# tyler-a-cox/fftvis

Hardware: AMD Instinct MI355X
Metric: simulated visibilities/sec (baselines x freqs x times) at eps=6e-8 (higher is better)
Workload: dtype f64; 1 GPU; C3: hera350, 100000 sources, 128 freqs, 20 times, 61075 baselines, polarized table beam, type3 NUFFT eps=6e-08 upsampfac=2

## Files before the change

### fftvis_amd/csrc/fv_nufft.h

```cpp
#pragma once

#include "fv_eskernel.h"

#include <hip/hip_ext.h>

#include <algorithm>
#include <cstdlib>
#include <array>
#include <map>
#include <memory>

namespace fv {

inline bool debug_switch_old_fft() {
    static const bool v = std::getenv("FFTVIS_HIP_OLD_FFT") != nullptr;
    return v;
}
inline bool debug_switch_natural_order() {
    static const bool v = std::getenv("FFTVIS_HIP_NATURAL_ORDER") != nullptr;
    return v;
}

constexpr int BINLOG = 3;
constexpr int GROUP = 16;
// ... 1987 lines not shown
    int64_t items_per_xcd;
    int n2[3], no[3];
    int P[3], cnt[3];
    double h[3];
    double btc[3], xc[3];
    int64_t out_fg_stride;
    int64_t out_k_stride;
    int64_t out_pol_off[16];
    int accumulate;
    int herm;
    int basis, kk, ll, nbasis, ncoef_freq, f_first;
    int transpose_flipped, basis_part, negate_all;
    const int *ctab;
    int ctab_stride, ncc;
    int *err;
    int wt_k;
    double wt_zc, wt_zh;
    const void *wt_bz;
    int zd_n;
    double zd_h, zd_btc, zd_xc;
    void *gs;
    int gs_nf, gs_f0;
    int64_t gs_nbls;
    const double *tg_w;
};

__device__ inline double bessel_j_series(int k, double x) {
    double lead = 1.0;
    for (int i = 1; i <= k; ++i) lead *= 0.5 * x / (double)i;
    const double q = -0.25 * x * x;
// ... 7 lines not shown
}

__device__ inline cplx<double> wterm_factor(int k, double zc, double zh, double zq) {
    double sn, cs;
    sincos(zc * zq, &sn, &cs);
    const double mag = (k ? 2.0 : 1.0) * bessel_j_series(k, zh * zq);
    const cplx<double> e = {cs * mag, sn * mag};
    switch (k & 3) {
        case 0: return e;
        case 1: return {-e.im, e.re};
        case 2: return {-e.re, -e.im};
        default: return {e.im, -e.re};
    }
}

template <typename T, int DIM, bool HERM, int NR, bool ZD = false, bool WT = false, bool GRAD = false, bool TANGENT = false>
__global__ __launch_bounds__(INTERP_THREADS) void k_interp(
    const cplx<T> *__restrict__ grid, int64_t N, const T *__restrict__ bt0,
    const T *__restrict__ bt1, const T *__restrict__ bt2, const int *__restrict__ bl_idx,
    const signed char *__restrict__ flip, const double *__restrict__ scale, InterpArgs a,
    KerParams ker, cplx<T> *__restrict__ out, const cplx<T> *__restrict__ coef,
    const int *__restrict__ ant1, const int *__restrict__ ant2, const int *__restrict__ ustart,
    const int *__restrict__ upairs) {
    const int tid = threadIdx.x;
    const int g = tid & (GROUP - 1);
    const int lane_base = (tid & 63) & ~(GROUP - 1);
    constexpr int IPW = INTERP_THREADS / GROUP;
    const int64_t per_xcd = a.items_per_xcd;
    const int64_t item = (int64_t)(blockIdx.x & 7) * per_xcd + (int64_t)(blockIdx.x >> 3) * IPW + tid / GROUP;
    if ((int64_t)(blockIdx.x >> 3) * IPW + tid / GROUP >= per_xcd || item >= N * a.nfg) return;
    const int fg = (int)(item / N);
// ... 48 lines not shown
    double pr = 1.0 / den, pi_ = 0.0;
    if (ph != 0.0) {
        double sn, cs;
        sincos(ph, &sn, &cs);
        pi_ = pr * sn;
        pr = pr * cs;
    }

    const int64_t row_sz = (int64_t)a.P[0] * a.cnt[0];
    const int64_t slab_sz = DIM == 2 && a.ctab ? row_sz * a.ncc : row_sz * a.P[1] * a.cnt[1];
    const int64_t plane_sz = DIM == 3 ? slab_sz * a.P[2] * a.cnt[2] : slab_sz;
    const int nouter = DIM == 3 ? w : 1;
    constexpr int NSIDE = HERM ? 2 : 1;
    constexpr int NVAL = HERM ? 2 : 16;
    double vre[NSIDE][HERM ? NVAL : 1], vim[NSIDE][HERM ? NVAL : 1];
    int j0s[NSIDE][DIM], roffs[NSIDE][NR], gcols[NSIDE];
    T kvs[NSIDE][DIM];
#pragma unroll
    for (int side = 0; side < NSIDE; ++side) {
        const double sgn = side ? -1.0 : 1.0;
        int (&j0)[DIM] = j0s[side];
        T (&kv)[DIM] = kvs[side];
#pragma unroll
        for (int d = 0; d < DIM; ++d) {
            const double e = sgn * th[d] * a.n2[d] * (0.5 / M_PI) + 0.5 * a.no[d];
            int j = (int)ceil(e - 0.5 * w);
            j = max(0, min(a.no[d] - w, j));
            j0[d] = j;
            kv[d] = g < w ? es_eval<T>((T)((double)(j + g) - e), beta, c4) : T(0);
        }
        int (&roff)[NR] = roffs[side];
        {
            const int P1 = a.P[1], c1 = a.cnt[1];
            int q1 = j0[1] / P1, r1 = j0[1] - q1 * P1;
#pragma unroll
            for (int rr = 0; rr < NR; ++rr) {
                int posr = r1 * c1 + q1;
                if (DIM == 2 && a.ctab) {
                    const int t = a.ctab[(int64_t)fg * a.ctab_stride + posr];
                    if (t == 0 && rr < w && g == 0 && a.err) atomicAdd(a.err, 1);
                    posr = max(t - 1, 0);
                }
                roff[rr] = posr * (int)row_sz;
                const int inc = rr + 1 < w ? 1 : 0;
                r1 += inc;
                const int wrap = r1 == P1 ? 1 : 0;
                r1 = wrap ? 0 : r1;
                q1 += wrap;
            }
        }
        gcols[side] = out_pos(min(j0[0] + g, a.no[0] - 1), a.P[0], a.cnt[0]);
    }
#pragma unroll
    for (int side = 0; side < NSIDE; ++side) {
        const double sgn = side ? -1.0 : 1.0;
        const int (&j0)[DIM] = j0s[side];
        const T (&kv)[DIM] = kvs[side];
        const int (&roff)[NR] = roffs[side];
        const int gcol = gcols[side];
        T k1[NR];
#pragma unroll
        for (int r = 0; r < NR; ++r) k1[r] = __shfl(kv[1], lane_base + r, 64);
        const double pis = side ? -pi_ : pi_;
        constexpr int RUNROLL = HERM ? NVAL : 1;
#pragma unroll RUNROLL
        for (int r = 0; r < (HERM ? NVAL : a.tpol); ++r) {
            const cplx<T> *plane = grid + ((int64_t)fg * a.tpol + r) * (zd ? plane_sz * a.zd_n : plane_sz) + gcol;
            T sr = T(0), si = T(0);
            if (zd) {
                double er, ei, dr, di;
                sincos(sgn * thz, &di, &dr);
                sincos(-sgn * thz * (double)(a.zd_n / 2), &ei, &er);
                double ar_ = 0.0, ai_ = 0.0;
                for (int zk = 0; zk < a.zd_n; ++zk) {
                    const cplx<T> *slab = plane + (int64_t)zk * plane_sz;
                    cplx<T> v[NR];
#pragma unroll
                    for (int rr = 0; rr < NR; ++rr) v[rr] = slab[roff[rr]];
                    T tr = T(0), ti = T(0);
#pragma unroll
                    for (int rr = 0; rr < NR; ++rr) {
                        tr += v[rr].re * k1[rr];
                        ti += v[rr].im * k1[rr];
                    }
                    ar_ += (double)tr * er - (double)ti * ei;
                    ai_ += (double)tr * ei + (double)ti * er;
                    const double e2 = er * dr - ei * di;
                    ei = er * di + ei * dr;
                    er = e2;
                }
                sr = (T)ar_;
                si = (T)ai_;
            }
            for (int ro = 0; ro < (zd ? 0 : nouter); ++ro) {
                T k2 = T(1);
                const cplx<T> *slab = plane;
                if (DIM == 3) {
                    k2 = __shfl(kv[DIM - 1], lane_base + ro, 64);
                    slab += (int64_t)out_pos(j0[DIM - 1] + ro, a.P[DIM - 1], a.cnt[DIM - 1]) * slab_sz;
                }
                cplx<T> v[NR];
#pragma unroll
                for (int rr = 0; rr < NR; ++rr) v[rr] = slab[roff[rr]];
                T tr = T(0), ti = T(0);
#pragma unroll
                for (int rr = 0; rr < NR; ++rr) {
                    tr += v[rr].re * k1[rr];
                    ti += v[rr].im * k1[rr];
                }
                sr += tr * k2;
                si += ti * k2;
            }
            sr *= kv[0];
            si *= kv[0];
#pragma unroll
            for (int off = GROUP / 2; off > 0; off >>= 1) {
                sr += __shfl_xor(sr, off, 64);
                si += __shfl_xor(si, off, 64);
            }
            const double vr0 = (double)sr * pr - (double)si * pis;
            const double vi0 = (double)sr * pis + (double)si * pr;
// ... 179 lines not shown
        }
      }
    }
}

struct RowMaskArgs {
    int w, nfg, sides;
    int n2x, nox, Px, cntx, n2y, noy, Py, Qy;
    double hx, btcx, hy, btcy;
    int blk_log, nblk, nw, ctab_stride;
};
template <typename T>
__global__ void k_plan_rowmask(int64_t NU, const T *__restrict__ btx, const T *__restrict__ bty,
                               const int *__restrict__ bl_idx, const signed char *__restrict__ flip,
                               const int *__restrict__ ustart, const double *__restrict__ scale, RowMaskArgs a,
                               const int *__restrict__ ctab, unsigned long long *__restrict__ mask) {
    const int64_t item = (int64_t)blockIdx.x * blockDim.x + threadIdx.x;
    if (item >= NU * a.nfg * a.sides) return;
    const int side = (int)(item % a.sides);
    const int64_t rest = item / a.sides;
    const int fg = (int)(rest / NU);
    const int64_t ui = rest % NU;
    const int64_t kl = ustart ? ustart[ui] : ui;
    const int64_t k = bl_idx ? bl_idx[kl] : kl;
    const double sg = (flip && flip[kl]) ? -1.0 : 1.0, sgn = side ? -1.0 : 1.0, sc = scale[fg];
    int lo[2], hi[2];
    const double hh[2] = {a.hx, a.hy}, bc[2] = {a.btcx, a.btcy};
    const int n2[2] = {a.n2x, a.n2y}, no[2] = {a.nox, a.noy};
    const double b[2] = {(double)btx[k], (double)bty[k]};
#pragma unroll
    for (int d = 0; d < 2; ++d) {
        const double sv = sc * sg * b[d];
        const double th = hh[d] * (sv - sc * bc[d]);
        const double e = sgn * th * n2[d] * (0.5 / M_PI) + 0.5 * no[d];
        const double t = e - 0.5 * a.w, jc = ceil(t);
        const bool amb = jc - t < 1e-6 || jc - t > 1.0 - 1e-6;
        lo[d] = max(0, min(no[d] - a.w, (int)jc));
        hi[d] = lo[d] + a.w - 1;
        if (amb) {
            lo[d] = max(0, lo[d] - 1);
            hi[d] = min(no[d] - 1, hi[d] + 1);
        }
    }
    const int half = a.noy / 2;
    for (int cx = lo[0]; cx <= hi[0]; ++cx) {
        const int t = ctab[(int64_t)fg * a.ctab_stride + out_pos(cx, a.Px, a.cntx)];
        if (!t) continue;
        const int64_t blk = (t - 1) >> a.blk_log;
        for (int cy = lo[1]; cy <= hi[1]; ++cy) {
            const int l = cy - half;
            int pp = l % a.Py;
            if (pp < 0) pp += a.Py;
            const int ks = (l - pp) / a.Py;
            const int c = (ks < 0 ? ks + a.Qy : ks) >> 4;
            atomicOr(&mask[(((int64_t)fg * a.nblk + blk) * a.Py + pp) * a.nw + (c >> 6)], 1ull << (c & 63));
        }
    }
}

struct BasisTerm {
    const void *coef;
    const int *ant1, *ant2;
    int kk, ll, nbasis, nfreq, f_first;
    int part = 0, negate = 0;
    void *gs = nullptr;
    int gs_nf = 0, gs_f0 = 0;
    int64_t gs_nbls = 0;
};

struct WTerm {
    int k;
    double zc, zh;
// ... 51 lines not shown
    }
    int *col_err = nullptr;
    const unsigned long long *col_omask = nullptr;
    int col_omask_nblk = 0;
    double col_out_cells = 0;
    void arm_columns(const int *tab, const int *xtab, int tpol, int ncc, int *err = nullptr, const unsigned long long *omask = nullptr,
                     int omask_nblk = 0) {
        col_tab = tab && xtab && (dim == 2 || zdirect) && b_block_log() ? tab : nullptr;
        col_xtab = col_tab ? xtab : nullptr;
        col_tab_tpol = tpol;
        col_ncc = ncc;
        col_err = err;
        col_omask = col_tab ? omask : nullptr;
        col_omask_nblk = omask_nblk;
        col_out_cells = 0;
    }
    int ypass_cols_log() const {
        int tpr, rpw;
        rowfft_shape(geo.d[1], true, tpr, rpw);
        return ilog2_c(rpw);
    }
    void build_rowmask(int64_t NU, const T *btx, const T *bty, const int *bl_idx, const signed char *flip, const int *ustart,
                       const double *scale_dev, int nfg, bool both, const int *ctab, int ncc, unsigned long long *mask,
                       int nblk, int nw) const {
        const DimGeom &x = geo.d[0], &y = geo.d[1];
        RowMaskArgs a{};
        a.w = ker.w;
        a.nfg = nfg;
        a.sides = both ? 2 : 1;
        a.n2x = x.n2; a.nox = x.no; a.Px = x.sP(); a.cntx = x.cnt(); a.hx = x.h; a.btcx = x.btc;
        a.n2y = y.n2; a.noy = y.no; a.Py = y.P; a.Qy = y.Q; a.hy = y.h; a.btcy = y.btc;
        a.blk_log = ypass_cols_log();
        a.nblk = nblk;
        a.nw = nw;
        a.ctab_stride = x.nos();
        (void)ncc;
        const int64_t items = NU * nfg * a.sides;
        if (items == 0) return;
        hipLaunchKernelGGL(k_plan_rowmask<T>, dim3((unsigned)cdiv(items, 256)), dim3(256), 0, stream, NU, btx, bty, bl_idx,
                           flip, ustart, scale_dev, a, ctab, mask);
    }
    int xcols() const { return col_tab ? col_ncc : geo.d[0].nos(); }
    int b_block_log_public() const { return b_block_log(); }
    bool columns_possible() const { return (dim == 2 || zdirect) && b_block_log() != 0 && y_reads_columns() && !fused_possible(); }
    bool fused_possible() const;
    bool prepare_fused_gather(int64_t N, const T *btx, const T *bty, const int *bl_idx, const signed char *flip,
                              const double *scale_dev, int nfg, int tpol, cplx<T> *out, int64_t out_fg_stride,
                              int64_t out_k_stride, const int64_t *out_pol_off, int64_t targets_serial = 0,
                              cplx<T> *out_mate = nullptr);
    int64_t M = 0;
    int64_t geom_serial = 0;

    DevBuf i0u, fu, tile_of, binmeta, bin_start, i0s, fs, perm, slot_id, kw, scan_tot, scan_off, scan_tot2, scan_off2;
    const int *Mp = nullptr;
    int *oob_ptr = nullptr;
// ... 329 lines not shown
    int launch_spread(int ntrans, int tbegin, hipEvent_t e0, hipEvent_t e1, Nufft3 *mate);
    void buffer_cells(int64_t &c0, int64_t &c1) const;
    void fft(int ntrans, Nufft3 *mate = nullptr);
    bool gang_compatible(const Nufft3 &o) const {
        bool ok = dim == 2 && o.dim == 2 && M == o.M && ker.w == o.ker.w;
        for (int d = 0; d < 2 && ok; ++d)
            ok = geo.d[d].na == o.geo.d[d].na && geo.d[d].n2 == o.geo.d[d].n2 && geo.d[d].no == o.geo.d[d].no &&
                 geo.d[d].h == o.geo.d[d].h && geo.d[d].xc == o.geo.d[d].xc && geo.d[d].btc == o.geo.d[d].btc;
        return ok;
    }
    double fft_traffic_cells() const;
    double fft_flops() const {
        const DimGeom &x = geo.d[0], &y = geo.d[1], &z = geo.d[2];
        const double zin = dim > 2 ? z.na : 1;
        auto f = [](const DimGeom &g) { return 5.0 * g.n2 * std::log2((double)g.n2); };
        double c = zin * y.na * f(x) + zin * (double)xcols() * f(y);
        if (dim > 2 && !zdirect) c += (double)x.nos() * y.nos() * f(z);
        return c;
    }
    int64_t spread_cells() const {
        return dim == 2 ? order_cells : row_ext_ptr ? order_cells * geo.d[2].na : geo.cells_a();
    }
    void interp(int64_t N, const T *btx, const T *bty, const T *btz, const int *bl_idx,
                const signed char *flip, const double *scale_dev, int nfg, int tpol,
                cplx<T> *out, int64_t out_fg_stride, int64_t out_k_stride,
                const int64_t *out_pol_off, bool accumulate, const struct BasisTerm *basis = nullptr,
                int herm = 0, const int *ustart = nullptr, int64_t nuniq = 0, const int *upairs = nullptr,
                const struct WTerm *wt = nullptr, const struct TanTerm *tan = nullptr);

   private:
    void rowfft(const cplx<T> *in, cplx<T> *out, const DimGeom &g, const cplx<T> *twd,
// ... 275 lines not shown
        FV_HIP(hipFuncSetAttribute(reinterpret_cast<const void *>(&k_rowfft_dif<T>),
                                   hipFuncAttributeMaxDynamicSharedMemorySize, 160 * 1024));
    hipLaunchKernelGGL(k_rowfft_dif<T>, jobs, dim3(a.tpr * a.rpw), smem, stream, in, out, twd, a);
}

template <typename T>
double Nufft3<T>::fft_traffic_cells() const {
    const DimGeom &x = geo.d[0], &y = geo.d[1], &z = geo.d[2];
    const double zin = dim > 2 ? z.na : 1;
    int tpr, rpw;
    rowfft_shape(y, true, tpr, rpw);
    const double xo = col_tab ? (double)col_ncc : (double)x.no;
    const double ain = row_ext_ptr ? (double)order_cells : (double)x.na * y.na;
    double c = zin * (ain + xo * y.na);
    if (!y_reads_columns()) c += zin * 2.0 * x.no * y.na;
    c += zin * (xo * y.na + (last_fft_fused ? 0.0 : col_tab && col_omask && col_out_cells > 0 ? col_out_cells : xo * y.no));
    if (dim > 2 && !zdirect) c += (double)x.no * y.no * (z.na + z.no);
    return c;
}

template <typename T>
void Nufft3<T>::fft(int ntrans, Nufft3 *mate) {
    const DimGeom &x = geo.d[0], &y = geo.d[1], &z = geo.d[2];
    int64_t c0, c1;
    buffer_cells(c0, c1);
    buf1.reserve(sizeof(cplx<T>) * c1 * ntrans);
    cplx<T> *cur = buf0.as<cplx<T>>(), *oth = buf1.as<cplx<T>>();
    cplx<T> *cur1 = nullptr, *oth1 = nullptr;
    if (mate) {
        FV_REQUIRE(gang_compatible(*mate), "gang launch needs two plans of one geometry");
        mate->buf1.reserve(sizeof(cplx<T>) * c1 * ntrans);
        cur1 = mate->buf0.template as<cplx<T>>();
        oth1 = mate->buf1.template as<cplx<T>>();
    }
    const int64_t zin = dim > 2 ? z.na : 1;
    const int64_t np = (int64_t)ntrans * zin;
    const int64_t xp = b_pitch();
    const int blk = b_block_log();
    FV_REQUIRE(!col_tab || (blk && y_reads_columns() && !fused_active), "column plan: blocked B, column-mode y-pass, stand-alone gather");
    first_pass_ext = row_ext_ptr;
    rowfft(cur, oth, x, tw_cur[0], np, y.na, (int64_t)y.na * x.na, x.na, 1, xp, 0, nullptr, cur1, oth1, 0, blk);
    first_pass_ext = nullptr;
    std::swap(cur, oth);
    std::swap(cur1, oth1);
    if (y_reads_columns()) {
        rowfft(cur, oth, y, tw_cur[1], np, xp, (int64_t)y.na * xp, 1, xp, 0, xcols(),
               fused_active ? &fused_args : nullptr, cur1, oth1, blk, 0);
        std::swap(cur, oth);
        std::swap(cur1, oth1);
    } else {
        dim3 tg((unsigned)cdiv(x.nos(), 32), (unsigned)cdiv(y.na, 32), (unsigned)np);
        hipLaunchKernelGGL(k_transpose<T>, tg, dim3(256), 0, stream, cur, oth, y.na, x.nos());
        if (mate) hipLaunchKernelGGL(k_transpose<T>, tg, dim3(256), 0, stream, cur1, oth1, y.na, x.nos());
        rowfft(oth, cur, y, tw_cur[1], np, x.nos(), (int64_t)x.nos() * y.na, y.na, 1, 0, 0, nullptr,
               oth1, cur1);
    }
    if (dim > 2 && !zdirect) {
        const int64_t nc = (int64_t)x.nos() * y.nos();
        rowfft(cur, oth, z, tw_cur[2], ntrans, nc, (int64_t)z.na * nc, 1, nc);
        std::swap(cur, oth);
// ... 153 lines not shown
        bt[i] = bts[map[i]];
    }
    FV_REQUIRE((int64_t)a.P[0] * a.cnt[0] * (col_tab ? (int64_t)col_ncc : (int64_t)a.P[1] * a.cnt[1]) < ((int64_t)1 << 31),
               "transform output slab of 2^31 elements or more: beyond the gather's 32-bit row offsets");
    a.out_fg_stride = out_fg_stride;
    a.out_k_stride = out_k_stride;
    for (int r = 0; r < 16; ++r) a.out_pol_off[r] = out_pol_off ? out_pol_off[r] : 0;
    a.accumulate = accumulate ? 1 : 0;
    if (col_tab) {
        FV_REQUIRE(gdim == 2, "column plan: 2-D transforms (or 3-D ones with the direct third dimension)");
        a.ctab = col_tab;
        a.ctab_stride = geo.d[0].nos();
        a.ncc = col_ncc;
        a.err = col_err;
    }
    a.herm = herm;
    a.transpose_flipped = transpose_flipped ? 1 : 0;
    a.wt_k = -1;
    if (wt) {
        FV_REQUIRE(dim == 2 && wt->bz && wt->k >= 0, "height terms ride on 2-D transforms");
        a.wt_k = wt->k;
        a.wt_zc = wt->zc;
        a.wt_zh = wt->zh;
        a.wt_bz = wt->bz;
    }
    const int64_t items = N * nfg;
    constexpr int IPW = INTERP_THREADS / GROUP;
    a.items_per_xcd = cdiv(cdiv(items, 8), IPW) * IPW;
    const dim3 grid((unsigned)(8 * (a.items_per_xcd / IPW)));
    const bool r9 = ker.w <= 9;
// ... 23 lines not shown
    }
    if (tan) {
        FV_REQUIRE(!basis && !a.gs, "tangent epilogue: no basis term and no gradient epilogue");
        a.tg_w = tan->w;
        kern = gdim == 2 ? (herm ? (r9 ? k_interp<T, 2, true, 9, false, false, false, true> : k_interp<T, 2, true, 16, false, false, false, true>)
                                 : (r9 ? k_interp<T, 2, false, 9, false, false, false, true> : k_interp<T, 2, false, 16, false, false, false, true>))
                         : (herm ? (r9 ? k_interp<T, 3, true, 9, false, false, false, true> : k_interp<T, 3, true, 16, false, false, false, true>)
                                 : (r9 ? k_interp<T, 3, false, 9, false, false, false, true> : k_interp<T, 3, false, 16, false, false, false, true>));
        if (zd)
            kern = herm ? (r9 ? k_interp<T, 2, true, 9, true, false, false, true> : k_interp<T, 2, true, 16, true, false, false, true>)
                        : (r9 ? k_interp<T, 2, false, 9, true, false, false, true> : k_interp<T, 2, false, 16, true, false, false, true>);
        if (wt)
            kern = herm ? (r9 ? k_interp<T, 2, true, 9, false, true, false, true> : k_interp<T, 2, true, 16, false, true, false, true>)
                        : (r9 ? k_interp<T, 2, false, 9, false, true, false, true> : k_interp<T, 2, false, 16, false, true, false, true>);
    }
    hipLaunchKernelGGL(kern, grid, dim3(INTERP_THREADS), 0, stream, (const cplx<T> *)grid_out, N, bt[0], bt[1], bt[2],
                       bl_idx, flip, scale_dev, a, ker, out, coef, ant1, ant2, ustart, upairs);
}

}
```

### fftvis_amd/csrc/fv_sim.h

```cpp
#pragma once

#include <atomic>
#include <chrono>
#include <cstdio>
#include <thread>
#include "fv_nufft.h"
#include <unordered_map>

#include <algorithm>
#include <array>
#include <cstdlib>
#include <memory>

namespace fv {

constexpr double SPEED_OF_LIGHT = 299792458.0;

struct BeamDesc {
    int kind;
    int order;
    double diameter;
    double js[8];
    double ps;
    const void *table;
// ... 1739 lines not shown
    int64_t out_f_stride = 0;
    int out_shared = 0;
    int adjoint_path = 0;
    int last_adjoint_path = 0;
    virtual void sync() = 0;
    virtual void stats(double *v, int n) = 0;
    virtual void reset_stats() = 0;
    virtual void enable_timing(int on) = 0;
    virtual void timing(double *ms, int n) = 0;
};

enum { TM_SPREAD = 0, TM_FFT, TM_INTERP, TM_STRENGTHS, TM_PREP, TM_COUNT };
enum {
    ST_SPREAD_LAUNCHES = 0, ST_SPREAD_CELLS, ST_SOURCE_VISITS, ST_FFT_CELLS, ST_GATHERED, ST_ABOVE_HORIZON, ST_N2X, ST_N2Y,
    ST_NA_XY, ST_W, ST_SIGMA, ST_MAX_ABOVE_HORIZON, ST_FFT_FLOPS, ST_N2_3, ST_NA_3, ST_HEIGHT_TERMS, ST_LANES, ST_LANE_MODE,
    ST_LIGHT_FROM, ST_LIGHTER_FROM
};

template <typename T>
class Sim : public SimBase {
    int device;
    hipStream_t stream = nullptr;
    double eps, sigma;
    double sigma_run = 2.0;
    bool polarized;
    int tpol;

    int64_t nsrc = 0;
    int nfreq_cat = 0;
    bool pol_sky = false;
    DevBuf d_eq, d_flux;

// ... 520 lines not shown

    struct ColPlan {
        int64_t serial;
        int pair, fa, fb, nos, sP, cnt, n2, no, w;
        double h, btc;
        bool both;
        DevBuf tab, xtab;
        int yna = 0, blk = 0;
        int ncc = 0;
        bool use = false;
        int yn2 = 0, yno = 0, yP = 0, yQ = 0;
        double yh = 0, ybtc = 0;
        DevBuf omask;
        int nblk = 0;
        double out_cells = 0;
    };
    std::vector<std::unique_ptr<ColPlan>> col_plans;
    std::vector<ColPlan *> col_plan_of[NCLS];
    ColPlan *column_plan(int pi, const Pair &pr, int fa, int fb, Nufft3<T> *n0) {
        const DimGeom &x = n0->geo.d[0], &y = n0->geo.d[1];
        const int w = n0->ker.w;
        const bool both = pr.herm || pr.mirror;
        for (auto &c : col_plans)
            if (c->serial == targets_serial && c->pair == pi && c->fa == fa && c->fb == fb && c->nos == x.nos() &&
                c->sP == x.sP() && c->cnt == x.cnt() && c->n2 == x.n2 && c->no == x.no && c->w == w && c->h == x.h &&
                c->btc == x.btc && c->both == both && c->yn2 == y.n2 && c->yno == y.no && c->yP == y.P && c->yQ == y.Q &&
                c->yh == y.h && c->ybtc == y.btc && c->yna == y.na && c->blk == n0->b_block_log_public())
                return c.get();
        std::unique_ptr<ColPlan> c(new ColPlan{targets_serial, pi, fa, fb, x.nos(), x.sP(), x.cnt(), x.n2, x.no, w, x.h, x.btc, both});
        const int nfg = fb - fa, stride = x.nos(), P = x.sP(), cnt = x.cnt();
        std::vector<int> tab((size_t)nfg * stride, 0);
        const int64_t nu = pr.h_ustart.empty() ? pr.n : (int64_t)pr.h_ustart.size() - 1;
        c->use = true;
        for (int fg = 0; fg < nfg && c->use; ++fg) {
            int *row = tab.data() + (size_t)fg * stride;
            const double sc = freqs[fa + fg];
            for (int64_t ui = 0; ui < nu; ++ui) {
                const int64_t kl = pr.h_ustart.empty() ? ui : pr.h_ustart[ui];
                const int64_t k = pr.h_idx[kl];
                const double sg = pr.h_flip[kl] ? -1.0 : 1.0;
                const double sv = sc * sg * (double)(T)h_bls[k];
                const double th = x.h * (sv - sc * x.btc);
                for (int side = 0; side < (both ? 2 : 1); ++side) {
                    const double e = (side ? -1.0 : 1.0) * th * x.n2 * (0.5 / M_PI) + 0.5 * x.no;
// ... 33 lines not shown
                FV_HIP(hipMemsetAsync(c->omask.p, 0, sizeof(unsigned long long) * words, stream));
                hipStream_t keep = n0->stream;
                n0->stream = stream;
                n0->build_rowmask(nu, d_bls.as<T>(), d_bls.as<T>() + nbls, pr.trivial ? nullptr : pr.idx->template as<int>(),
                                  pr.trivial ? nullptr : pr.flip->template as<signed char>(),
                                  pr.ustart ? pr.ustart->template as<int>() : nullptr, d_freqs.as<double>() + fa, nfg, both,
                                  c->tab.template as<int>(), c->ncc, c->omask.template as<unsigned long long>(), c->nblk, nw);
                n0->stream = keep;
                std::vector<unsigned long long> hm(words);
                FV_HIP(hipMemcpyAsync(hm.data(), c->omask.p, sizeof(unsigned long long) * words, hipMemcpyDeviceToHost, stream));
                FV_HIP(hipStreamSynchronize(stream));
                double bits = 0;
                for (unsigned long long v : hm) bits += __builtin_popcountll(v);
                c->out_cells = bits * 16.0 * (1 << bl) / nfg;
            }
        }
        col_plans.push_back(std::move(c));
        return col_plans.back().get();
    }

    void set_basis(int nant, int K, int nfreq, const void *coefs, const int *ant1,
                   const int *ant2) override {
        FV_HIP(hipSetDevice(device));
        FV_REQUIRE(polarized, "basis beams need a polarized engine (wrapper.py:280-283)");
        FV_REQUIRE(nbls > 0 && K >= 1 && K == (int)beams.size(), "set_array and the K basis beams first");
        FV_REQUIRE(nfreq == (int)freqs.size(), "beam_coefs frequency axis != freqs");
        for (int64_t b = 0; b < nbls; ++b)
            FV_REQUIRE(ant1[b] >= 0 && ant1[b] < nant && ant2[b] >= 0 && ant2[b] < nant, "antenna index out of range");
        nbasis = K;
        nant_basis = nant;
// ... 634 lines not shown
            double term = a;
            while (term > 0.1 * eps && K < 64) {
                ++K;
                term *= 0.5 * a / K;
            }
            const char *ek = std::getenv("FFTVIS_HIP_WTERM_MAX");
            if (K <= (ek ? std::atoi(ek) : 16)) {
                r.K = K;
                r.zc = r.xc[2];
                r.zh = r.X[2];
                r.a = a;
            }
        }
        r.D = r.K ? 2 : dim();
        st[ST_HEIGHT_TERMS] = r.K;
    }
    void light_classes(RunPlan &r) {
        r.k0 = 0;
        r.k1 = r.K;
        if (r.K >= 3 && sizeof(T) == 8 && this->sigma == 2.0 && !std::getenv("FFTVIS_HIP_NO_WTERM_LIGHT")) {
            std::vector<double> ck(r.K);
            double c = 1.0;
            for (int k = 0; k < r.K; ++k) {
                ck[k] = (k ? 2.0 : 1.0) * c;
                c *= 0.5 * r.a / (k + 1);
            }
            for (int k0 = 1; k0 + 2 <= r.K; ++k0) {
                double sl = 0;
                for (int k = k0; k < r.K; ++k) sl += ck[k];
                const double el = 0.3 * eps / sl;
// ... 322 lines not shown
                        }
                        ev_end(e1, ls);
                        if (!(strengths_ahead && &grp == &groups.front() && &pr == first_pair && kt == 0))
                            launch_strengths(L, r, pr, fa, nfg, M, Mps[m], ls, kt, nf_, tu + m);
                    }
                    const int nmom = r.moments ? 3 : 0;
                    const int nrounds = std::max(1, r.nsets());
                    for (int rd = 0; rd < nrounds; ++rd) {
                    for (int m = 0; m < nm; ++m) {
                        Nufft3<T> *P = Ls[m]->plan[c].get();
                        P->strengths_off = r.nsets() ? (int64_t)rd * P->M * ntrans : 0;
                        P->arm_columns(on ? cp->tab.template as<int>() : nullptr, on ? cp->xtab.template as<int>() : nullptr, tg,
                                       on ? cp->ncc : 0, d_err.as<int>() + 3,
                                       on && cp->omask.p ? cp->omask.template as<unsigned long long>() : nullptr, on ? cp->nblk : 0);
                        P->col_out_cells = on && cp->omask.p ? cp->out_cells : 0.0;
                    }
                    {
                    RoctxRange rr("spread");
                    if (timing_level >= 2 || (timing_level == 1 && sampled)) {
                        const size_t e3 = ev_slot(TM_SPREAD);
                        nufft->spread(ntrans, ev_pool[e3].a, ev_pool[e3].b, mate);
                        spread_timed += nm;
                    } else if (ride_heavy_done && pipe && &grp == &groups.back() && &pr == last_pair && kt + 1 >= std::max(1, r.K) &&
                               rd + 1 == nrounds) {
                        nufft->spread(ntrans, nullptr, L0.heavy_done, mate);
                        heavy_recorded = true;
                    } else {
                        nufft->spread(ntrans, nullptr, nullptr, mate);
                    }
                    }
// ... 1133 lines not shown
```

### fftvis_amd/gpu/gpu_simulate.py

```python

from __future__ import annotations

import ctypes
import atexit
import logging
import warnings

import numpy as np

from .. import _lib
from ..core import utils
from ..core.antenna_gridding import check_antpos_griddability
from ..core.beams import (airy_factors, checked_spline_order, describe_beam, feed_index, is_sampled_analytic,
                          table_tolerance)
from ..core.coords import SiderealRotation, eq_unit_vectors, julian_dates
from ..core.simulate import SimulationEngine, default_accuracy_dict

logger = logging.getLogger(__name__)


_IDLE_HANDLES: dict = {}
atexit.register(lambda: release_handles())


# ... 207 lines not shown
        _lib.check(self._L.fv_sim_run_source_adjoint(self._h, t0, t1, f0, f1, gp, g_dev, tp, t_dev, int(bool(accumulate))))

    def run_tangent(self, t0, t1, f0, f1, dbls, dtopo, out):
        bp, b_dev = _buffer_addr(dbls)
        tp, t_dev = _buffer_addr(dtopo)
        op, o_dev = _buffer_addr(out)
        _lib.check(self._L.fv_sim_run_tangent(self._h, t0, t1, f0, f1, bp, b_dev, tp, t_dev, op, o_dev))

    def run_device(self, t0, t1, f0, f1, out_ptr):
        _lib.check(self._L.fv_sim_run(self._h, t0, t1, f0, f1, _lib.ptr(out_ptr), 1))

    def sync(self):
        _lib.check(self._L.fv_sim_sync(self._h))

    def stats(self):
        v = np.zeros(20)
        _lib.check(self._L.fv_sim_stats(self._h, _lib.ptr(v), 20))
        keys = ["spread_launches", "spread_cells", "source_visits", "fft_cells", "interp_items",
                "sources_above_horizon", "n2x", "n2y", "n2z", "w", "upsample_used", "max_above_horizon", "fft_flops",
                "n2_3", "na_3", "height_terms", "lanes", "lane_mode", "height_terms_light_from", "height_terms_lighter_from"]
        return dict(zip(keys, v))

    def reset_stats(self):
        _lib.check(self._L.fv_sim_reset_stats(self._h))

    def enable_timing(self, on=True):
        _lib.check(self._L.fv_sim_enable_timing(self._h, int(on)))

    def timing(self):
        v = np.zeros(6)
        _lib.check(self._L.fv_sim_timing(self._h, _lib.ptr(v), 6))
        return dict(zip(["spread", "fft", "interp", "strengths", "prep", "spread_launches_timed"], v))


def register_with_reference() -> bool:
# ... 409 lines not shown
```

Baseline: 191.3 million visibilities/s.

## Contract x-direction interpolation into unique baseline-coordinate columns before the y FFT

Adds a contraction step in the 2-D column plan. Before the y-pass FFT, the w x-taps of the spreading kernel are applied once for each unique baseline x coordinate, so the y FFT runs over nhp contracted columns rather than every occupied x column. Interpolation then reads a single column per baseline side instead of NR rows. This needs a host-side planning pass with synchronisations, extra plan buffers and a new LDS-staged contraction kernel. The feature is gated by an environment variable and a compile-time default, so it may be inactive.

```diff
diff --git a/fftvis_amd/csrc/fv_nufft.h b/fftvis_amd/csrc/fv_nufft.h
--- a/fftvis_amd/csrc/fv_nufft.h
+++ b/fftvis_amd/csrc/fv_nufft.h
@@ -2025,6 +2025,7 @@
     const int *ctab;
     int ctab_stride, ncc;
     int *err;
+    const int *hcol;
     int wt_k;
     double wt_zc, wt_zh;
     const void *wt_bz;
@@ -2062,7 +2063,8 @@
     }
 }
 
-template <typename T, int DIM, bool HERM, int NR, bool ZD = false, bool WT = false, bool GRAD = false, bool TANGENT = false>
+template <typename T, int DIM, bool HERM, int NR, bool ZD = false, bool WT = false, bool GRAD = false, bool TANGENT = false,
+          bool XC = false>
 __global__ __launch_bounds__(INTERP_THREADS) void k_interp(
     const cplx<T> *__restrict__ grid, int64_t N, const T *__restrict__ bt0,
     const T *__restrict__ bt1, const T *__restrict__ bt2, const int *__restrict__ bl_idx,
@@ -2141,7 +2143,8 @@
     constexpr int NSIDE = HERM ? 2 : 1;
     constexpr int NVAL = HERM ? 2 : 16;
     double vre[NSIDE][HERM ? NVAL : 1], vim[NSIDE][HERM ? NVAL : 1];
-    int j0s[NSIDE][DIM], roffs[NSIDE][NR], gcols[NSIDE];
+    constexpr int NRL = XC ? 1 : NR;
+    int j0s[NSIDE][DIM], roffs[NSIDE][NRL], gcols[NSIDE];
     T kvs[NSIDE][DIM];
 #pragma unroll
     for (int side = 0; side < NSIDE; ++side) {
@@ -2156,8 +2159,10 @@
             j0[d] = j;
             kv[d] = g < w ? es_eval<T>((T)((double)(j + g) - e), beta, c4) : T(0);
         }
-        int (&roff)[NR] = roffs[side];
-        {
+        int (&roff)[NRL] = roffs[side];
+        if constexpr (XC) {
+            roff[0] = a.hcol[2 * ui + (HERM ? side : (a.negate_all != 0 ? 1 : 0))] * (int)row_sz;
+        } else {
             const int P1 = a.P[1], c1 = a.cnt[1];
             int q1 = j0[1] / P1, r1 = j0[1] - q1 * P1;
 #pragma unroll
@@ -2183,11 +2188,11 @@
         const double sgn = side ? -1.0 : 1.0;
         const int (&j0)[DIM] = j0s[side];
         const T (&kv)[DIM] = kvs[side];
-        const int (&roff)[NR] = roffs[side];
+        const int (&roff)[NRL] = roffs[side];
         const int gcol = gcols[side];
-        T k1[NR];
-#pragma unroll
-        for (int r = 0; r < NR; ++r) k1[r] = __shfl(kv[1], lane_base + r, 64);
+        T k1[NRL];
+#pragma unroll
+        for (int r = 0; r < NRL; ++r) k1[r] = XC ? T(1) : __shfl(kv[1], lane_base + r, 64);
         const double pis = side ? -pi_ : pi_;
         constexpr int RUNROLL = HERM ? NVAL : 1;
 #pragma unroll RUNROLL
@@ -2201,12 +2206,12 @@
                 double ar_ = 0.0, ai_ = 0.0;
                 for (int zk = 0; zk < a.zd_n; ++zk) {
                     const cplx<T> *slab = plane + (int64_t)zk * plane_sz;
-                    cplx<T> v[NR];
-#pragma unroll
-                    for (int rr = 0; rr < NR; ++rr) v[rr] = slab[roff[rr]];
+                    cplx<T> v[NRL];
+#pragma unroll
+                    for (int rr = 0; rr < NRL; ++rr) v[rr] = slab[roff[rr]];
                     T tr = T(0), ti = T(0);
 #pragma unroll
-                    for (int rr = 0; rr < NR; ++rr) {
+                    for (int rr = 0; rr < NRL; ++rr) {
                         tr += v[rr].re * k1[rr];
                         ti += v[rr].im * k1[rr];
                     }
@@ -2226,12 +2231,12 @@
                     k2 = __shfl(kv[DIM - 1], lane_base + ro, 64);
                     slab += (int64_t)out_pos(j0[DIM - 1] + ro, a.P[DIM - 1], a.cnt[DIM - 1]) * slab_sz;
                 }
-                cplx<T> v[NR];
-#pragma unroll
-                for (int rr = 0; rr < NR; ++rr) v[rr] = slab[roff[rr]];
+                cplx<T> v[NRL];
+#pragma unroll
+                for (int rr = 0; rr < NRL; ++rr) v[rr] = slab[roff[rr]];
                 T tr = T(0), ti = T(0);
 #pragma unroll
-                for (int rr = 0; rr < NR; ++rr) {
+                for (int rr = 0; rr < NRL; ++rr) {
                     tr += v[rr].re * k1[rr];
                     ti += v[rr].im * k1[rr];
                 }
@@ -2441,7 +2446,8 @@
 __global__ void k_plan_rowmask(int64_t NU, const T *__restrict__ btx, const T *__restrict__ bty,
                                const int *__restrict__ bl_idx, const signed char *__restrict__ flip,
                                const int *__restrict__ ustart, const double *__restrict__ scale, RowMaskArgs a,
-                               const int *__restrict__ ctab, unsigned long long *__restrict__ mask) {
+                               const int *__restrict__ ctab, unsigned long long *__restrict__ mask,
+                               const int *__restrict__ hcol = nullptr) {
     const int64_t item = (int64_t)blockIdx.x * blockDim.x + threadIdx.x;
     if (item >= NU * a.nfg * a.sides) return;
     const int side = (int)(item % a.sides);
@@ -2470,8 +2476,9 @@
         }
     }
     const int half = a.noy / 2;
+    if (hcol) lo[0] = hi[0] = 0;
     for (int cx = lo[0]; cx <= hi[0]; ++cx) {
-        const int t = ctab[(int64_t)fg * a.ctab_stride + out_pos(cx, a.Px, a.cntx)];
+        const int t = hcol ? 1 + hcol[2 * ui + side] : ctab[(int64_t)fg * a.ctab_stride + out_pos(cx, a.Px, a.cntx)];
         if (!t) continue;
         const int64_t blk = (t - 1) >> a.blk_log;
         for (int cy = lo[1]; cy <= hi[1]; ++cy) {
@@ -2483,6 +2490,116 @@
             atomicOr(&mask[(((int64_t)fg * a.nblk + blk) * a.Py + pp) * a.nw + (c >> 6)], 1ull << (c & 63));
         }
     }
+}
+
+constexpr int XC_GROUP = 16, XC_ROWS = 16, XC_WMAX = 16, XC_MAXSRC = 40;
+struct ContractPlanArgs {
+    int w, nfg, nh, nhp, ngrp, blk;
+    int n2, no, P, cnt, ctab_stride;
+    double h, btc;
+};
+template <typename T>
+__global__ void k_plan_contract(const double *__restrict__ coord, const double *__restrict__ scale, ContractPlanArgs a,
+                                KerParams ker, const int *__restrict__ ctab, T *__restrict__ wt, int *__restrict__ slot,
+                                int *__restrict__ src, int *__restrict__ nsrc, int *__restrict__ maxsrc, int *err) {
+    const int item = blockIdx.x * blockDim.x + threadIdx.x;
+    if (item >= a.nfg * a.ngrp) return;
+    const int fg = item / a.ngrp, q = item % a.ngrp;
+    const double sc = scale[fg];
+    const T beta = (T)ker.beta, c4 = (T)ker.c;
+    const int w = a.w, nb = 1 << a.blk;
+    int *srcq = src + (int64_t)item * XC_MAXSRC;
+    int ns = 0;
+    for (int hl = 0; hl < XC_GROUP; ++hl) {
+        const int hc = q * XC_GROUP + hl;
+        if (hc >= a.nhp) break;
+        T *wq = wt + ((int64_t)fg * a.nhp + hc) * XC_WMAX;
+        int *sq = slot + ((int64_t)fg * a.nhp + hc) * XC_WMAX;
+        for (int rr = 0; rr < XC_WMAX; ++rr) {
+            wq[rr] = T(0);
+            sq[rr] = 0;
+        }
+        if (hc >= a.nh) continue;
+        const double sv = sc * coord[hc];
+        const double th = a.h * (sv - sc * a.btc);
+        const double e = th * a.n2 * (0.5 / M_PI) + 0.5 * a.no;
+        int j = (int)ceil(e - 0.5 * w);
+        j = max(0, min(a.no - w, j));
+        for (int rr = 0; rr < w; ++rr) {
+            const int t = ctab[(int64_t)fg * a.ctab_stride + out_pos(j + rr, a.P, a.cnt)];
+            if (t == 0) {
+                if (err) atomicAdd(err, 1);
+                continue;
+            }
+            const int cc = t - 1, b = cc >> a.blk;
+            int s = 0;
+            while (s < ns && s < XC_MAXSRC && srcq[s] != b) ++s;
+            if (s == ns) {
+                if (ns < XC_MAXSRC) srcq[ns] = b;
+                ++ns;
+            }
+            if (s >= XC_MAXSRC) continue;
+            wq[rr] = es_eval<T>((T)((double)(j + rr) - e), beta, c4);
+            sq[rr] = s * XC_ROWS * nb + (cc & (nb - 1));
+        }
+    }
+    nsrc[item] = min(ns, XC_MAXSRC);
+    atomicMax(maxsrc, ns);
+}
+
+template <typename T>
+struct ContractArgs {
+    int w, tpol, nh, nhp, ngrp, blk, na_y, ntiles;
+    int64_t b_plane, h_plane;
+    const T *wt;
+    const int *slot, *src, *nsrc;
+    const cplx<T> *in1;
+    cplx<T> *out1;
+};
+template <typename T>
+__global__ __launch_bounds__(256) void k_contract_cols(const cplx<T> *__restrict__ in, cplx<T> *__restrict__ out,
+                                                        ContractArgs<T> a) {
+    extern __shared__ __align__(16) unsigned char xc_smem[];
+    const int nb = 1 << a.blk, tile = XC_ROWS << a.blk;
+    T *lw = (T *)xc_smem;
+    int *ls = (int *)(lw + XC_GROUP * XC_WMAX);
+    using V = T __attribute__((ext_vector_type(2)));
+    V *lb = (V *)(ls + XC_GROUP * XC_WMAX);
+    const int tid = threadIdx.x;
+    const int q = blockIdx.x % a.ngrp, r0 = (blockIdx.x / a.ngrp) * XC_ROWS;
+    const int64_t p = blockIdx.y;
+    const int fg = (int)(p / a.tpol);
+    const V *bp = reinterpret_cast<const V *>(blockIdx.z ? a.in1 : in) + p * a.b_plane;
+    V *hp = reinterpret_cast<V *>(blockIdx.z ? a.out1 : out) + p * a.h_plane;
+    const int item = fg * a.ngrp + q;
+    const int ns = a.nsrc[item];
+    const int *srcq = a.src + (int64_t)item * XC_MAXSRC;
+    const int hc0 = q * XC_GROUP;
+    {
+        const int hl = tid >> 4, rr = tid & 15, hc = hc0 + hl;
+        const bool in_ = hc < a.nhp;
+        lw[tid] = in_ ? a.wt[((int64_t)fg * a.nhp + hc) * XC_WMAX + rr] : T(0);
+        ls[tid] = in_ ? a.slot[((int64_t)fg * a.nhp + hc) * XC_WMAX + rr] : 0;
+    }
+    const int rows_left = a.na_y - r0;
+    for (int i = tid; i < ns * tile; i += 256) {
+        const int s = i / tile, rem = i - s * tile;
+        V v = {T(0), T(0)};
+        if ((rem >> a.blk) < rows_left) v = bp[((int64_t)srcq[s] * a.na_y + r0) * nb + rem];
+        lb[i] = v;
+    }
+    __syncthreads();
+    const int c = tid & (nb - 1), r = (tid >> a.blk) & (XC_ROWS - 1), hl = (tid >> (a.blk + 4)) * nb + c, hc = hc0 + hl;
+    if (hl >= XC_GROUP || hc >= a.nhp || r >= rows_left) return;
+    V acc = {T(0), T(0)};
+    if (hc < a.nh) {
+        for (int rr = 0; rr < a.w; ++rr) {
+            const T wv = lw[hl * XC_WMAX + rr];
+            if (wv == T(0)) continue;
+            acc += wv * lb[ls[hl * XC_WMAX + rr] + r * nb];
+        }
+    }
+    hp[((int64_t)(hc >> a.blk) * a.na_y + r0 + r) * nb + c] = acc;
 }
 
 struct BasisTerm {
@@ -2564,7 +2681,41 @@
         col_omask = col_tab ? omask : nullptr;
         col_omask_nblk = omask_nblk;
         col_out_cells = 0;
-    }
+        xc = XContract{};
+    }
+    struct XContract {
+        const int *hcol = nullptr, *slot = nullptr, *src = nullptr, *nsrc = nullptr;
+        const T *wt = nullptr;
+        int nh = 0, nhp = 0, maxsrc = 0;
+        const unsigned long long *omask = nullptr;
+        int omask_nblk = 0;
+        double out_cells = 0;
+    } xc;
+    void arm_xcontract(const XContract &x) {
+        FV_REQUIRE(!x.hcol || (col_tab && dim == 2), "contracted footprints ride on a 2-D column plan");
+        xc = x;
+    }
+    static size_t contract_lds_bytes(int maxsrc, int blk) {
+        return (size_t)XC_GROUP * XC_WMAX * (sizeof(T) + sizeof(int)) + (size_t)maxsrc * (XC_ROWS << blk) * sizeof(cplx<T>);
+    }
+    void build_contract(const double *coord, int nh, int nhp, const double *scale_dev, int nfg, const int *ctab, T *wt,
+                        int *slot, int *src, int *nsrc, int *maxsrc, int *err) const {
+        const DimGeom &x = geo.d[0];
+        ContractPlanArgs a{};
+        a.w = ker.w;
+        a.nfg = nfg;
+        a.nh = nh;
+        a.nhp = nhp;
+        a.ngrp = (int)cdiv(nhp, XC_GROUP);
+        a.blk = b_block_log();
+        a.n2 = x.n2; a.no = x.no; a.P = x.sP(); a.cnt = x.cnt(); a.ctab_stride = x.nos();
+        a.h = x.h; a.btc = x.btc;
+        const int items = nfg * a.ngrp;
+        if (items == 0) return;
+        hipLaunchKernelGGL(k_plan_contract<T>, dim3((unsigned)cdiv(items, 64)), dim3(64), 0, stream, coord, scale_dev, a, ker,
+                           ctab, wt, slot, src, nsrc, maxsrc, err);
+    }
+    int ycols() const { return xc.hcol ? xc.nhp : xcols(); }
     int ypass_cols_log() const {
         int tpr, rpw;
         rowfft_shape(geo.d[1], true, tpr, rpw);
@@ -2572,7 +2723,7 @@
     }
     void build_rowmask(int64_t NU, const T *btx, const T *bty, const int *bl_idx, const signed char *flip, const int *ustart,
                        const double *scale_dev, int nfg, bool both, const int *ctab, int ncc, unsigned long long *mask,
-                       int nblk, int nw) const {
+                       int nblk, int nw, const int *hcol = nullptr) const {
         const DimGeom &x = geo.d[0], &y = geo.d[1];
         RowMaskArgs a{};
         a.w = ker.w;
@@ -2588,7 +2739,7 @@
         const int64_t items = NU * nfg * a.sides;
         if (items == 0) return;
         hipLaunchKernelGGL(k_plan_rowmask<T>, dim3((unsigned)cdiv(items, 256)), dim3(256), 0, stream, NU, btx, bty, bl_idx,
-                           flip, ustart, scale_dev, a, ctab, mask);
+                           flip, ustart, scale_dev, a, ctab, mask, hcol);
     }
     int xcols() const { return col_tab ? col_ncc : geo.d[0].nos(); }
     int b_block_log_public() const { return b_block_log(); }
@@ -2948,7 +3099,7 @@
         const DimGeom &x = geo.d[0], &y = geo.d[1], &z = geo.d[2];
         const double zin = dim > 2 ? z.na : 1;
         auto f = [](const DimGeom &g) { return 5.0 * g.n2 * std::log2((double)g.n2); };
-        double c = zin * y.na * f(x) + zin * (double)xcols() * f(y);
+        double c = zin * y.na * f(x) + zin * (double)ycols() * f(y);
         if (dim > 2 && !zdirect) c += (double)x.nos() * y.nos() * f(z);
         return c;
     }
@@ -3254,6 +3405,11 @@
     const double ain = row_ext_ptr ? (double)order_cells : (double)x.na * y.na;
     double c = zin * (ain + xo * y.na);
     if (!y_reads_columns()) c += zin * 2.0 * x.no * y.na;
+    if (xc.hcol) {
+        c += zin * (xo * y.na + (double)xc.nhp * y.na);
+        c += zin * ((double)xc.nhp * y.na + (xc.omask && xc.out_cells > 0 ? xc.out_cells : (double)xc.nhp * y.no));
+        return c;
+    }
     c += zin * (xo * y.na + (last_fft_fused ? 0.0 : col_tab && col_omask && col_out_cells > 0 ? col_out_cells : xo * y.no));
     if (dim > 2 && !zdirect) c += (double)x.no * y.no * (z.na + z.no);
     return c;
@@ -3283,7 +3439,40 @@
     first_pass_ext = nullptr;
     std::swap(cur, oth);
     std::swap(cur1, oth1);
-    if (y_reads_columns()) {
+    if (xc.hcol) {
+        FV_REQUIRE(col_tab && blk && dim == 2 && !fused_active && y_reads_columns(), "contracted footprints: 2-D column plan");
+        ContractArgs<T> ca{};
+        ca.w = ker.w;
+        ca.tpol = col_tab_tpol;
+        ca.nh = xc.nh;
+        ca.nhp = xc.nhp;
+        ca.ngrp = (int)cdiv(xc.nhp, XC_GROUP);
+        ca.blk = blk;
+        ca.na_y = y.na;
+        ca.ntiles = (int)cdiv(y.na, XC_ROWS);
+        ca.b_plane = (int64_t)y.na * xp;
+        ca.h_plane = (int64_t)y.na * xc.nhp;
+        ca.wt = xc.wt;
+        ca.slot = xc.slot;
+        ca.src = xc.src;
+        ca.nsrc = xc.nsrc;
+        ca.in1 = cur1;
+        ca.out1 = oth1;
+        FV_REQUIRE(np <= 65535, "contracted footprints: too many planes in one launch");
+        hipLaunchKernelGGL(k_contract_cols<T>, dim3((unsigned)(ca.ngrp * ca.ntiles), (unsigned)np, mate ? 2 : 1), dim3(256),
+                           contract_lds_bytes(xc.maxsrc, blk), stream, (const cplx<T> *)cur, oth, ca);
+        std::swap(cur, oth);
+        std::swap(cur1, oth1);
+        const unsigned long long *keep_mask = col_omask;
+        const int keep_nblk = col_omask_nblk;
+        col_omask = xc.omask;
+        col_omask_nblk = xc.omask_nblk;
+        rowfft(cur, oth, y, tw_cur[1], np, xc.nhp, (int64_t)y.na * xc.nhp, 1, xc.nhp, 0, xc.nhp, nullptr, cur1, oth1, blk, 0);
+        col_omask = keep_mask;
+        col_omask_nblk = keep_nblk;
+        std::swap(cur, oth);
+        std::swap(cur1, oth1);
+    } else if (y_reads_columns()) {
         rowfft(cur, oth, y, tw_cur[1], np, xp, (int64_t)y.na * xp, 1, xp, 0, xcols(),
                fused_active ? &fused_args : nullptr, cur1, oth1, blk, 0);
         std::swap(cur, oth);
@@ -3467,6 +3656,12 @@
         a.ncc = col_ncc;
         a.err = col_err;
     }
+    const bool xcg = xc.hcol != nullptr;
+    if (xcg) {
+        FV_REQUIRE(col_tab && dim == 2 && !(basis && basis->gs) && !tan, "contracted footprints: forward gathers of a 2-D column plan");
+        a.hcol = xc.hcol;
+        a.ncc = xc.nhp;
+    }
     a.herm = herm;
     a.transpose_flipped = transpose_flipped ? 1 : 0;
     a.wt_k = -1;
@@ -3520,6 +3715,13 @@
             kern = herm ? (r9 ? k_interp<T, 2, true, 9, false, true, false, true> : k_interp<T, 2, true, 16, false, true, false, true>)
                         : (r9 ? k_interp<T, 2, false, 9, false, true, false, true> : k_interp<T, 2, false, 16, false, true, false, true>);
     }
+    if (xcg) {
+        kern = herm ? (r9 ? k_interp<T, 2, true, 9, false, false, false, false, true> : k_interp<T, 2, true, 16, false, false, false, false, true>)
+                    : (r9 ? k_interp<T, 2, false, 9, false, false, false, false, true> : k_interp<T, 2, false, 16, false, false, false, false, true>);
+        if (wt)
+            kern = herm ? (r9 ? k_interp<T, 2, true, 9, false, true, false, false, true> : k_interp<T, 2, true, 16, false, true, false, false, true>)
+                        : (r9 ? k_interp<T, 2, false, 9, false, true, false, false, true> : k_interp<T, 2, false, 16, false, true, false, false, true>);
+    }
     hipLaunchKernelGGL(kern, grid, dim3(INTERP_THREADS), 0, stream, (const cplx<T> *)grid_out, N, bt[0], bt[1], bt[2],
                        bl_idx, flip, scale_dev, a, ker, out, coef, ant1, ant2, ustart, upairs);
 }
diff --git a/fftvis_amd/csrc/fv_sim.h b/fftvis_amd/csrc/fv_sim.h
--- a/fftvis_amd/csrc/fv_sim.h
+++ b/fftvis_amd/csrc/fv_sim.h
@@ -1777,8 +1777,12 @@
 enum {
     ST_SPREAD_LAUNCHES = 0, ST_SPREAD_CELLS, ST_SOURCE_VISITS, ST_FFT_CELLS, ST_GATHERED, ST_ABOVE_HORIZON, ST_N2X, ST_N2Y,
     ST_NA_XY, ST_W, ST_SIGMA, ST_MAX_ABOVE_HORIZON, ST_FFT_FLOPS, ST_N2_3, ST_NA_3, ST_HEIGHT_TERMS, ST_LANES, ST_LANE_MODE,
-    ST_LIGHT_FROM, ST_LIGHTER_FROM
+    ST_LIGHT_FROM, ST_LIGHTER_FROM, ST_XCONTRACT_COLS
 };
+
+#ifndef FV_XCONTRACT_DEFAULT
+#define FV_XCONTRACT_DEFAULT 0
+#endif
 
 template <typename T>
 class Sim : public SimBase {
@@ -2329,7 +2333,81 @@
         DevBuf omask;
         int nblk = 0;
         double out_cells = 0;
+        DevBuf hcol, xcoord, xwt, xslot, xsrc, xnsrc, xomask;
+        int nh = 0, nhp = 0, xmaxsrc = 0, xnblk = 0;
+        double xout_cells = 0;
+        bool xuse = false, xwanted = false;
     };
+    static bool xcontract_wanted() {
+        if (std::getenv("FFTVIS_HIP_NO_XCONTRACT")) return false;
+        const char *e = std::getenv("FFTVIS_HIP_XCONTRACT");
+        return e ? std::atoi(e) != 0 : FV_XCONTRACT_DEFAULT != 0;
+    }
+    void contract_plan(ColPlan &c, const Pair &pr, int64_t nu, int nfg, Nufft3<T> *n0) {
+        const DimGeom &y = n0->geo.d[1];
+        const int b = c.blk;
+        if (n0->dim != 2 || (b != 2 && b != 3) || c.w > XC_WMAX) return;
+        std::vector<double> key((size_t)nu * 2, 0.0), uniq;
+        const int ns = c.both ? 2 : 1;
+        uniq.reserve((size_t)nu * ns);
+        for (int64_t ui = 0; ui < nu; ++ui) {
+            const int64_t kl = pr.h_ustart.empty() ? ui : pr.h_ustart[ui];
+            const double v = (pr.h_flip[kl] ? -1.0 : 1.0) * (double)(T)h_bls[pr.h_idx[kl]];
+            for (int sd = 0; sd < ns; ++sd) {
+                const double k = (sd ? -v : v) + 0.0;
+                key[(size_t)ui * 2 + sd] = k;
+                uniq.push_back(k);
+            }
+        }
+        std::sort(uniq.begin(), uniq.end());
+        uniq.erase(std::unique(uniq.begin(), uniq.end()), uniq.end());
+        c.nh = (int)uniq.size();
+        c.nhp = (c.nh + 7) / 8 * 8;
+        if (c.nh == 0 || c.nhp * 2 > c.ncc) return;
+        std::vector<int> hc((size_t)nu * 2, 0);
+        for (int64_t ui = 0; ui < nu; ++ui)
+            for (int sd = 0; sd < ns; ++sd)
+                hc[(size_t)ui * 2 + sd] = (int)(std::lower_bound(uniq.begin(), uniq.end(), key[(size_t)ui * 2 + sd]) - uniq.begin());
+        upload(c.hcol, hc.data(), sizeof(int) * hc.size(), 0);
+        upload(c.xcoord, uniq.data(), sizeof(double) * uniq.size(), 0);
+        const int ngrp = (c.nhp + XC_GROUP - 1) / XC_GROUP;
+        const size_t ncol = (size_t)nfg * c.nhp, ngq = (size_t)nfg * ngrp;
+        c.xwt.reserve(sizeof(T) * ncol * XC_WMAX);
+        c.xslot.reserve(sizeof(int) * ncol * XC_WMAX);
+        c.xsrc.reserve(sizeof(int) * ngq * XC_MAXSRC);
+        c.xnsrc.reserve(sizeof(int) * (ngq + 1));
+        FV_HIP(hipMemsetAsync(c.xsrc.p, 0, sizeof(int) * ngq * XC_MAXSRC, stream));
+        FV_HIP(hipMemsetAsync(c.xnsrc.p, 0, sizeof(int) * (ngq + 1), stream));
+        hipStream_t keep = n0->stream;
+        n0->stream = stream;
+        n0->build_contract(c.xcoord.template as<double>(), c.nh, c.nhp, d_freqs.as<double>() + c.fa, nfg, c.tab.template as<int>(),
+                           c.xwt.template as<T>(), c.xslot.template as<int>(), c.xsrc.template as<int>(), c.xnsrc.template as<int>(),
+                           c.xnsrc.template as<int>() + ngq, d_err.as<int>() + 3);
+        int maxsrc = 0;
+        FV_HIP(hipMemcpyAsync(&maxsrc, c.xnsrc.template as<int>() + ngq, sizeof(int), hipMemcpyDeviceToHost, stream));
+        FV_HIP(hipStreamSynchronize(stream));
+        c.xmaxsrc = maxsrc;
+        c.xuse = maxsrc >= 1 && maxsrc <= XC_MAXSRC && Nufft3<T>::contract_lds_bytes(maxsrc, b) <= 48 * 1024;
+        if (c.xuse && c.omask.p) {
+            const int bl = n0->ypass_cols_log(), nw = y.Q > 1024 ? y.Q / 1024 : 1;
+            c.xnblk = (c.nhp + (1 << bl) - 1) >> bl;
+            const size_t words = (size_t)nfg * c.xnblk * y.P * nw;
+            c.xomask.reserve(sizeof(unsigned long long) * words);
+            FV_HIP(hipMemsetAsync(c.xomask.p, 0, sizeof(unsigned long long) * words, stream));
+            n0->build_rowmask(nu, d_bls.as<T>(), d_bls.as<T>() + nbls, pr.trivial ? nullptr : pr.idx->template as<int>(),
+                              pr.trivial ? nullptr : pr.flip->template as<signed char>(),
+                              pr.ustart ? pr.ustart->template as<int>() : nullptr, d_freqs.as<double>() + c.fa, nfg, c.both,
+                              c.tab.template as<int>(), c.nhp, c.xomask.template as<unsigned long long>(), c.xnblk, nw,
+                              c.hcol.template as<int>());
+            std::vector<unsigned long long> hm(words);
+            FV_HIP(hipMemcpyAsync(hm.data(), c.xomask.p, sizeof(unsigned long long) * words, hipMemcpyDeviceToHost, stream));
+            FV_HIP(hipStreamSynchronize(stream));
+            double bits = 0;
+            for (unsigned long long v : hm) bits += __builtin_popcountll(v);
+            c.xout_cells = bits * 16.0 * (1 << bl) / nfg;
+        }
+        n0->stream = keep;
+    }
     std::vector<std::unique_ptr<ColPlan>> col_plans;
     std::vector<ColPlan *> col_plan_of[NCLS];
     ColPlan *column_plan(int pi, const Pair &pr, int fa, int fb, Nufft3<T> *n0) {
@@ -2340,9 +2418,11 @@
             if (c->serial == targets_serial && c->pair == pi && c->fa == fa && c->fb == fb && c->nos == x.nos() &&
                 c->sP == x.sP() && c->cnt == x.cnt() && c->n2 == x.n2 && c->no == x.no && c->w == w && c->h == x.h &&
                 c->btc == x.btc && c->both == both && c->yn2 == y.n2 && c->yno == y.no && c->yP == y.P && c->yQ == y.Q &&
-                c->yh == y.h && c->ybtc == y.btc && c->yna == y.na && c->blk == n0->b_block_log_public())
+                c->yh == y.h && c->ybtc == y.btc && c->yna == y.na && c->blk == n0->b_block_log_public() &&
+                c->xwanted == xcontract_wanted())
                 return c.get();
         std::unique_ptr<ColPlan> c(new ColPlan{targets_serial, pi, fa, fb, x.nos(), x.sP(), x.cnt(), x.n2, x.no, w, x.h, x.btc, both});
+        c->xwanted = xcontract_wanted();
         const int nfg = fb - fa, stride = x.nos(), P = x.sP(), cnt = x.cnt();
         std::vector<int> tab((size_t)nfg * stride, 0);
         const int64_t nu = pr.h_ustart.empty() ? pr.n : (int64_t)pr.h_ustart.size() - 1;
@@ -2406,6 +2486,7 @@
                 for (unsigned long long v : hm) bits += __builtin_popcountll(v);
                 c->out_cells = bits * 16.0 * (1 << bl) / nfg;
             }
+            if (c->xwanted) contract_plan(*c, pr, nu, nfg, n0);
         }
         col_plans.push_back(std::move(c));
         return col_plans.back().get();
@@ -3070,6 +3151,7 @@
         }
         r.D = r.K ? 2 : dim();
         st[ST_HEIGHT_TERMS] = r.K;
+        st[ST_XCONTRACT_COLS] = 0;
     }
     void light_classes(RunPlan &r) {
         r.k0 = 0;
@@ -3422,6 +3504,22 @@
                                        on ? cp->ncc : 0, d_err.as<int>() + 3,
                                        on && cp->omask.p ? cp->omask.template as<unsigned long long>() : nullptr, on ? cp->nblk : 0);
                         P->col_out_cells = on && cp->omask.p ? cp->out_cells : 0.0;
+                        if (on && cp->xuse && !gs && !r.tan_w && xcontract_wanted()) {
+                            typename Nufft3<T>::XContract x;
+                            x.hcol = cp->hcol.template as<int>();
+                            x.slot = cp->xslot.template as<int>();
+                            x.src = cp->xsrc.template as<int>();
+                            x.nsrc = cp->xnsrc.template as<int>();
+                            x.wt = cp->xwt.template as<T>();
+                            x.nh = cp->nh;
+                            x.nhp = cp->nhp;
+                            x.maxsrc = cp->xmaxsrc;
+                            x.omask = cp->xomask.p ? cp->xomask.template as<unsigned long long>() : nullptr;
+                            x.omask_nblk = cp->xnblk;
+                            x.out_cells = cp->xout_cells;
+                            P->arm_xcontract(x);
+                            st[ST_XCONTRACT_COLS] = cp->nhp;
+                        }
                     }
                     {
                     RoctxRange rr("spread");
diff --git a/fftvis_amd/gpu/gpu_simulate.py b/fftvis_amd/gpu/gpu_simulate.py
--- a/fftvis_amd/gpu/gpu_simulate.py
+++ b/fftvis_amd/gpu/gpu_simulate.py
@@ -245,11 +245,12 @@
         _lib.check(self._L.fv_sim_sync(self._h))
 
     def stats(self):
-        v = np.zeros(20)
-        _lib.check(self._L.fv_sim_stats(self._h, _lib.ptr(v), 20))
+        v = np.zeros(21)
+        _lib.check(self._L.fv_sim_stats(self._h, _lib.ptr(v), 21))
         keys = ["spread_launches", "spread_cells", "source_visits", "fft_cells", "interp_items",
                 "sources_above_horizon", "n2x", "n2y", "n2z", "w", "upsample_used", "max_above_horizon", "fft_flops",
-                "n2_3", "na_3", "height_terms", "lanes", "lane_mode", "height_terms_light_from", "height_terms_lighter_from"]
+                "n2_3", "na_3", "height_terms", "lanes", "lane_mode", "height_terms_light_from", "height_terms_lighter_from",
+                "xcontract_cols"]
         return dict(zip(keys, v))
 
     def reset_stats(self):
```

Measured after the change: 194.5 million visibilities/s (median of 6 runs). 1.7% higher.
